# ecmwf/anemoi-models

Hardware: AMD Instinct MI355X
Metric: mesh-node updates/sec (fwd step) (higher is better)
Workload: dtype bf16; 1 GPU; N320->ico-6, 16 GT blocks, 1024 ch, batch 1, 2 x 90 input vars -> 80 output vars, full encoder+processor+decoder forward; mesh_nodes=40962, grid_nodes=542080, processor_blocks=16, rollout_steps=1, parallelism=single GPU, device=AMD Radeon Graphics

## Files before the change

anemoi_models_amd/_lib.py:

```python

from __future__ import annotations

import ctypes
import os
from ctypes import c_char_p
from ctypes import c_float
from ctypes import c_int
from ctypes import c_int64
from ctypes import c_uint32
from ctypes import c_void_p

import torch

_PKG_DIR = os.path.dirname(os.path.abspath(__file__))
LIB_PATH = os.path.join(_PKG_DIR, "lib", "libanemoi_amd.so")

ANEMOI_OK = 0
ANEMOI_ERR_INVALID = 1
ANEMOI_ERR_UNSUPPORTED = 2
ANEMOI_ERR_LAUNCH = 3

F32 = 0
BF16 = 1

ACT_NONE, ACT_GELU, ACT_SILU, ACT_RELU = 0, 1, 2, 3
ACT_CODES = {"Identity": ACT_NONE, "GELU": ACT_GELU, "SiLU": ACT_SILU, "ReLU": ACT_RELU}

ABI_VERSION = 43


class GtBlockArgs(ctypes.Structure):

    _fields_ = [
        ("struct_bytes", c_int64), ("n_dst", c_int64),
        ("dtype", ctypes.c_int32), ("C", ctypes.c_int32), ("H", ctypes.c_int32), ("up", ctypes.c_int32),
        ("hidden", ctypes.c_int32), ("act", ctypes.c_int32), ("k_proj", ctypes.c_int32), ("n_in", ctypes.c_int32),
        ("eps_mlp", c_float), ("eps_out", c_float),
        ("x", c_void_p), ("ldx", c_int64), ("x_stats", c_void_p),
        ("w_in", c_void_p), ("b_in", c_void_p), ("cs_in", c_void_p),
        ("sq", c_void_p), ("ld_sq", c_int64),
        ("q", c_void_p), ("k", c_void_p), ("v", c_void_p), ("x_r", c_void_p), ("u", c_void_p),
        ("ldq", c_int64), ("ldkv", c_int64), ("ldr", c_int64), ("ldu", c_int64),
        ("edge_attr", c_void_p), ("rowptr", c_void_p), ("col", c_void_p),
        ("att", c_void_p), ("ld_att", c_int64),
        ("w_proj", c_void_p), ("b_proj", c_void_p), ("res", c_void_p), ("ld_res", c_int64), ("y", c_void_p),
        ("y_stats", c_void_p),
        ("w_fc1", c_void_p), ("b_fc1", c_void_p), ("cs_fc1", c_void_p), ("h", c_void_p),
        ("w_fc2", c_void_p), ("b_fc2", c_void_p), ("out", c_void_p), ("out_stats", c_void_p),
        ("stats_ws", c_void_p), ("stats_ws_bytes", c_int64),
        ("run_ptr", c_void_p), ("run_perm", c_void_p), ("n_runs", c_int64),
        ("sched", c_void_p), ("sched_slots", ctypes.c_int32), ("sched_steps", ctypes.c_int32), ("n_src", c_int64),
        ("run_dst", c_void_p), ("n_edges", c_int64),
        ("tile_hdr", c_void_p), ("tile_dst", c_void_p), ("tile_src", c_void_p), ("tile_slot", c_void_p), ("tile_xcd", c_void_p),
        ("tile_max_per_xcd", ctypes.c_int32), ("tile_src_cap", ctypes.c_int32), ("tile_edge_cap", ctypes.c_int32),
        ("tile_pad", ctypes.c_int32),
    ]

class TfmBlockArgs(ctypes.Structure):

    _fields_ = [
        ("struct_bytes", c_int64), ("rows", c_int64),
        ("dtype", ctypes.c_int32), ("B", ctypes.c_int32), ("S", ctypes.c_int32), ("C", ctypes.c_int32), ("H", ctypes.c_int32),
        ("hidden", ctypes.c_int32), ("act", ctypes.c_int32), ("window", ctypes.c_int32),
        ("eps1", c_float), ("eps2", c_float),
        ("dropout_p", c_float), ("dropout_seed", c_uint32), ("dropout_seed_dev", c_void_p),
        ("dropout_h0", ctypes.c_int32), ("dropout_h_total", ctypes.c_int32),
        ("x", c_void_p), ("ldx", c_int64),
        ("ln1_w", c_void_p), ("ln1_b", c_void_p), ("ln2_w", c_void_p), ("ln2_b", c_void_p),
        ("w_qkv", c_void_p), ("b_qkv", c_void_p), ("w_proj", c_void_p), ("b_proj", c_void_p),
        ("w_fc1", c_void_p), ("b_fc1", c_void_p), ("w_fc2", c_void_p), ("b_fc2", c_void_p),
        ("h_ln", c_void_p), ("qkv", c_void_p), ("att", c_void_p), ("y", c_void_p), ("h", c_void_p),
        ("mhsa_ws", c_void_p), ("out", c_void_p),
    ]


SIGNATURES = {
    "anemoi_abi_version": (c_int, []),
    "anemoi_build_info": (ctypes.c_char_p, []),
    "anemoi_last_error": (c_char_p, []),
    "anemoi_layer_norm": (c_int, [c_int, c_void_p, c_int64, c_void_p, c_void_p, c_void_p, c_int64, c_int64, c_int,
                                  c_float, c_void_p]),
    "anemoi_layer_norm_residual": (c_int, [c_int, c_void_p, c_int64, c_void_p, c_void_p, c_void_p, c_int64, c_void_p, c_int64,
                                           c_int64, c_int, c_float, c_void_p]),
    "anemoi_layer_norm_stats": (c_int, [c_int, c_void_p, c_int64, c_void_p, c_void_p, c_void_p, c_int64, c_void_p, c_int64,
                                        c_int, c_float, c_void_p]),
    "anemoi_linear": (c_int, [c_int, c_int, c_void_p, c_int64, c_void_p, c_void_p, c_void_p, c_int64, c_void_p,
                              c_int64, c_int64, c_int, c_int, c_int, c_void_p]),
    "anemoi_linear_stats": (c_int, [c_int, c_void_p, c_int64, c_void_p, c_void_p, c_void_p, c_void_p, c_void_p, c_int64,
                                    c_void_p, c_int64, c_int64, c_int, c_int, c_void_p, c_int64, c_float, c_void_p,
                                    c_void_p]),
    "anemoi_row_stats": (c_int, [c_int, c_void_p, c_int64, c_void_p, c_int64, c_int, c_float, c_void_p]),
    "anemoi_linear_ln": (c_int, [c_int, c_int, c_void_p, c_int64, c_void_p, c_void_p, c_void_p, c_void_p, c_void_p,
                                 c_int64, c_void_p, c_int64, c_int64, c_int, c_int, c_int, c_void_p]),
    "anemoi_edge_attr_csr": (c_int, [c_void_p, c_int, c_void_p, c_int, c_int64, c_void_p, c_void_p, c_int, c_int,
                                     c_int64, c_void_p]),
    "anemoi_gt_edge_attention_folded": (c_int, [c_int, c_void_p, c_int64, c_void_p, c_void_p, c_int64, c_void_p,
                                                c_int64, c_void_p, c_int64, c_void_p, c_int, c_void_p, c_void_p,
                                                c_void_p, c_int64, c_void_p, c_int64, c_int, c_int, c_void_p]),
    "anemoi_gt_edge_attention_folded_runs": (c_int, [c_int, c_void_p, c_int64, c_void_p, c_void_p, c_int64, c_void_p,
                                                     c_int64, c_void_p, c_int64, c_void_p, c_int, c_void_p, c_void_p,
                                                     c_void_p, c_void_p, c_int64, c_void_p, c_int64, c_void_p, c_int64, c_int,
                                                     c_int, c_void_p]),
    "anemoi_gt_edge_attention_folded_groups": (c_int, [c_int, c_void_p, c_int64, c_void_p, c_void_p, c_int64, c_void_p,
                                                       c_int64, c_void_p, c_int64, c_void_p, c_int, c_void_p, c_void_p,
                                                       c_void_p, c_void_p, c_void_p, c_int64, c_int64, c_void_p, c_int64,
                                                       c_void_p, c_int64, c_int, c_int, c_void_p]),
    "anemoi_edge_schedule_shape": (c_int, [c_int, c_int64, c_int, c_void_p, c_void_p]),
    "anemoi_gt_edge_attention_folded_sched": (c_int, [c_int, c_void_p, c_int64, c_void_p, c_void_p, c_int64, c_void_p,
                                                      c_int64, c_void_p, c_int64, c_void_p, c_int, c_void_p, c_void_p,
                                                      c_void_p, c_int, c_int, c_int64, c_int64, c_void_p, c_int64, c_void_p,
                                                      c_int64, c_int, c_int, c_void_p]),
    "anemoi_gt_edge_attention_folded_tiles": (c_int, [c_int, c_void_p, c_int64, c_void_p, c_void_p, c_int64, c_void_p,
                                                      c_int64, c_void_p, c_int64, c_void_p, c_int, c_void_p, c_void_p,
                                                      c_void_p, c_void_p, c_void_p, c_void_p, c_void_p, c_int, c_int, c_int,
                                                      c_int64, c_int64, c_void_p, c_int64, c_void_p, c_int64, c_int, c_int,
                                                      c_void_p]),
    "anemoi_linear_dual": (c_int, [c_int, c_void_p, c_int64, c_void_p, c_void_p, c_void_p, c_int64, c_void_p, c_int64,
                                   c_int64, c_int, c_int, c_int, c_void_p]),
    "anemoi_linear_actgrad": (c_int, [c_int, c_void_p, c_int64, c_void_p, c_void_p, c_int64, c_void_p, c_int64, c_int64,
                                      c_int, c_int, c_int, c_void_p]),
    "anemoi_gt_conv": (c_int, [c_int, c_void_p, c_int64, c_void_p, c_void_p, c_int64, c_void_p, c_int64, c_void_p, c_int64,
                               c_void_p, c_void_p, c_void_p, c_int64, c_void_p, c_int64, c_int, c_int, c_float, c_uint32,
                               c_void_p, c_void_p]),
    "anemoi_gt_conv_backward_dst": (c_int, [c_int, c_void_p, c_int64, c_void_p, c_void_p, c_int64, c_void_p, c_int64,
                                            c_void_p, c_int64, c_void_p, c_void_p, c_void_p, c_void_p, c_void_p, c_void_p,
                                            c_void_p, c_int64, c_int64, c_int, c_int, c_float, c_uint32, c_void_p,
                                            c_void_p]),
    "anemoi_gt_conv_backward_src": (c_int, [c_int, c_void_p, c_int64, c_void_p, c_int64, c_void_p, c_void_p, c_void_p,
                                            c_void_p, c_void_p, c_void_p, c_void_p, c_void_p, c_int64, c_void_p, c_int64,
                                            c_int64, c_int, c_int, c_float, c_uint32, c_void_p, c_void_p]),
    "anemoi_gt_edge_attention": (c_int, [c_int, c_void_p, c_int64, c_void_p, c_void_p, c_int64, c_void_p, c_int64,
                                         c_void_p, c_int, c_int, c_void_p, c_void_p, c_void_p, c_void_p, c_void_p,
                                         c_int64, c_int64, c_int, c_int, c_void_p]),
    "anemoi_gather_add_act": (c_int, [c_int, c_void_p, c_int64, c_void_p, c_int64, c_void_p, c_int64, c_void_p, c_void_p,
                                      c_void_p, c_int64, c_int64, c_int, c_int, c_void_p]),
    "anemoi_segment_sum": (c_int, [c_int, c_void_p, c_int64, c_void_p, c_void_p, c_int64, c_int64, c_int, c_void_p]),
    "anemoi_segment_sum_cat": (c_int, [c_int, c_void_p, c_int64, c_void_p, c_void_p, c_int64, c_void_p, c_int64, c_int64,
                                       c_int, c_void_p]),
    "anemoi_mhsa_workspace_bytes": (c_int64, [c_int, c_int, c_int, c_int, c_int]),
    "anemoi_mhsa": (c_int, [c_int, c_void_p, c_int64, c_void_p, c_int64, c_void_p, c_void_p, c_int, c_int, c_int, c_int,
                            c_int, c_float, c_uint32, c_void_p, c_int, c_int, c_void_p]),
    "anemoi_mhsa_backward_workspace_bytes": (c_int64, [c_int, c_int, c_int, c_int, c_int]),
    "anemoi_mhsa_backward": (c_int, [c_int, c_void_p, c_int64, c_void_p, c_int64, c_void_p, c_int64, c_void_p, c_void_p,
                                     c_void_p, c_int64, c_void_p, c_int, c_int, c_int, c_int, c_int, c_float, c_uint32,
                                     c_void_p, c_int, c_int, c_void_p]),
    "anemoi_assemble_nodes": (c_int, [c_int, c_void_p, c_int, c_int, c_int, c_int64, c_int, c_void_p, c_int,
                                      c_void_p, c_int, c_void_p, c_int64, c_void_p, c_void_p, c_void_p]),
    "anemoi_finalize_output": (c_int, [c_void_p, c_int, c_void_p, c_int, c_int, c_int, c_int64, c_int, c_void_p,
                                       c_void_p, c_void_p, c_void_p, c_void_p, c_void_p]),
    "anemoi_assemble_node_rows": (c_int, [c_int, c_void_p, c_int, c_int64, c_int, c_void_p, c_int, c_void_p, c_int,
                                          c_void_p, c_int64, c_void_p, c_int64, c_void_p, c_void_p, c_void_p]),
# ... 96 lines not shown
```

anemoi_models_amd/csrc/elementwise.hip:

```cpp
#include <cstdlib>

#include "common.hpp"

namespace anemoi {

template <typename T>
__device__ __forceinline__ float round_to(float v);
template <>
__device__ __forceinline__ float round_to<float>(float v) { return v; }
template <>
__device__ __forceinline__ float round_to<bf16_t>(float v) { return bf16_to_f32(f32_to_bf16(v)); }

template <typename T, int VEC, int ITEMS>
__global__ __launch_bounds__(256) void layer_norm_kernel(const T* __restrict__ x, int64_t ldx,
                                                         const float* __restrict__ gamma,
                                                         const float* __restrict__ beta, T* __restrict__ y,
                                                         int64_t ldy, int64_t rows, int C, float eps,
                                                         float2* __restrict__ stats, const T* __restrict__ res = nullptr,
                                                         int64_t ldr = 0) {
  const int lane = threadIdx.x & 63;
  const int64_t row = (int64_t)blockIdx.x * 4 + (threadIdx.x >> 6);
  if (row >= rows) return;
  const T* xr = x + row * ldx;
  float v[ITEMS][VEC];
// ... 747 lines not shown
  hipLaunchKernelGGL(advance_input_kernel, dim3(flat_grid(total)), dim3(256), 0, as_stream(stream), x, B, T, Ens, G,
                     V_in, y, V_out, forcing, F, colmap);
  return check_launch("anemoi_advance_input");
}

static int finalize_output_impl(float* y, int V_out, const float* x, int B, int T, int Ens, int64_t G, int V_in,
                                const int32_t* src, const float* in_mul, const float* in_add, const float* out_mul,
                                const float* out_add, const int64_t* rows, int64_t n_rows, anemoi_stream_t stream) {
  ANEMOI_REQUIRE(y && x && src && B > 0 && T > 0 && Ens > 0 && G >= 0 && V_in > 0 && V_out > 0, ANEMOI_ERR_INVALID,
                 "anemoi_finalize_output: bad argument");
  ANEMOI_REQUIRE((in_mul == nullptr) == (in_add == nullptr) && (out_mul == nullptr) == (out_add == nullptr),
                 ANEMOI_ERR_INVALID, "anemoi_finalize_output: mul and add come together");
  const int64_t total = (rows != nullptr ? n_rows : (int64_t)B * Ens * G) * V_out;
  if (total == 0) return ANEMOI_OK;
  if (!force_idx64() && total < ((int64_t)1 << 31) - ((int64_t)1 << 24))
    hipLaunchKernelGGL(finalize_output_kernel<true>, dim3(flat_grid(total)), dim3(256), 0, as_stream(stream), y, V_out, x, B,
                       T, Ens, G, V_in, src, in_mul, in_add, out_mul, out_add, rows, n_rows);
  else
    hipLaunchKernelGGL(finalize_output_kernel<false>, dim3(flat_grid(total)), dim3(256), 0, as_stream(stream), y, V_out, x, B,
                       T, Ens, G, V_in, src, in_mul, in_add, out_mul, out_add, rows, n_rows);
  return check_launch("anemoi_finalize_output");
}

int anemoi_finalize_output(float* y, int V_out, const float* x, int B, int T, int Ens, int64_t G, int V_in,
                           const int32_t* src, const float* in_mul, const float* in_add, const float* out_mul,
                           const float* out_add, anemoi_stream_t stream) {
  return finalize_output_impl(y, V_out, x, B, T, Ens, G, V_in, src, in_mul, in_add, out_mul, out_add, nullptr, 0, stream);
}

int anemoi_finalize_output_rows(float* y, int V_out, const float* x, int T, int64_t G, int V_in, const int32_t* src,
                                const int64_t* rows, int64_t n_rows, const float* in_mul, const float* in_add,
                                const float* out_mul, const float* out_add, anemoi_stream_t stream) {
  ANEMOI_REQUIRE(n_rows >= 0 && (rows != nullptr || n_rows == 0), ANEMOI_ERR_INVALID,
                 "anemoi_finalize_output_rows: null row list");
  if (n_rows == 0) return ANEMOI_OK;
  return finalize_output_impl(y, V_out, x, 1, T, 1, G, V_in, src, in_mul, in_add, out_mul, out_add, rows, n_rows, stream);
}

int anemoi_bound_output(float* y, int V_out, int64_t rows, int n_ops, const int32_t* op_col, const float* op_lo,
                        const float* op_hi, const int32_t* op_mul, int n_fin, const int32_t* fin_col,
                        const float* fin_mul, const float* fin_add, anemoi_stream_t stream) {
  ANEMOI_REQUIRE(y && V_out > 0 && rows >= 0 && n_ops >= 0 && n_fin >= 0, ANEMOI_ERR_INVALID,
                 "anemoi_bound_output: bad argument");
  ANEMOI_REQUIRE(n_ops == 0 || (op_col && op_lo && op_hi && op_mul), ANEMOI_ERR_INVALID,
                 "anemoi_bound_output: null op list");
  ANEMOI_REQUIRE(n_fin == 0 || (fin_col && fin_mul && fin_add), ANEMOI_ERR_INVALID,
                 "anemoi_bound_output: null de-normalisation list");
  if (rows == 0 || (n_ops == 0 && n_fin == 0)) return ANEMOI_OK;
  hipLaunchKernelGGL(bound_output_kernel, dim3(flat_grid(rows)), dim3(256), 0, as_stream(stream), y, V_out, rows, n_ops,
                     op_col, op_lo, op_hi, op_mul, n_fin, fin_col, fin_mul, fin_add);
  return check_launch("anemoi_bound_output");
}

int anemoi_abi_version(void) { return 43; }

#ifndef ANEMOI_HIPCC_VERSION
#define ANEMOI_HIPCC_VERSION "unknown (built without anemoi_models_amd/_build.py)"
#endif
const char* anemoi_build_info(void) { return "gfx950; " ANEMOI_HIPCC_VERSION; }

const char* anemoi_last_error(void) { return err_buf(); }

}
```

anemoi_models_amd/layers/block.py:

```python

from __future__ import annotations

import os
from abc import ABC
from abc import abstractmethod
from typing import Optional

import torch
from torch import Tensor
from torch import nn

from .. import ops
from .. import runtime
from .. import training
from ..runtime import EdgePlan
from .conv import GraphConv
from .conv import GraphTransformerConv
from .mlp import MLP
from .mlp import NativeSequential
from .mlp import activation_class
from .mlp import fused_activation_name
from .mlp import linear_native


# ... 522 lines not shown
    ):
        if _group_size(model_comm_group) > 1:
            assert batch_size == 1, "Only batch size of 1 is supported when model is sharded across GPUs"
            return self._sharded(x, edge_attr, edge_index, shapes, batch_size, model_comm_group, size), edge_attr
        if training.wants_grad(self, x, edge_attr):
            return training.gt_processor_block(self, x, edge_attr, edge_index, size)
        dtype = runtime.compute_dtype(x)
        n = x.shape[0]
        if size is not None and tuple(size) != (n, n):
            raise ValueError(f"Encountered tensor with size {n} in dimension 0, but expected size {tuple(size)}")
        plan, ea = self._edge_inputs(edge_attr, edge_index, n, n, dtype)
        return self.native(_as_compute(x, dtype), ea, plan), edge_attr


class GraphTransformerMapperBlock(GraphTransformerBaseBlock):

    def __init__(
        self,
        in_channels: int,
        hidden_dim: int,
        out_channels: int,
        edge_dim: int,
        num_heads: int = 16,
        bias: bool = True,
        activation: str = "GELU",
        num_chunks: int = 1,
        update_src_nodes: bool = False,
        **kwargs,
    ) -> None:
        super().__init__(
            in_channels=in_channels, hidden_dim=hidden_dim, out_channels=out_channels, edge_dim=edge_dim,
            num_heads=num_heads, bias=bias, activation=activation, num_chunks=num_chunks,
            update_src_nodes=update_src_nodes, **kwargs,
        )
        self.layer_norm2 = nn.LayerNorm(in_channels)

    mx_node_mlp = True

    def native(self, x_src: Tensor, x_dst: Tensor, edge_attr_csr: Tensor, plan: EdgePlan, num_chunks: int = 1,
               halo=None, out_stats_eps: Optional[float] = None):
        dtype = x_dst.dtype
        self._check_channels(dtype)
        mx = runtime.mxfp8_enabled(dtype) and self.mx_node_mlp
        if mx:
            self._mx_check(self.node_dst_mlp[1].in_features if isinstance(self.node_dst_mlp[1], nn.Linear) else 0, halo)
        c = self.num_heads * self.out_channels_conv
        h_dst = x_dst.h if isinstance(x_dst, EmbeddedRows) else x_dst
        if isinstance(x_src, EmbeddedRows) and x_src.h is None and self.update_src_nodes:
            raise ValueError("update_src_nodes needs the embedded source rows")
        kv_layers, sq_layers = [self.lin_key, self.lin_value], [self.lin_self, self.lin_query]
        kv_args = ("kv", lambda: self._cat_linear("kv", kv_layers, dtype), lambda: self._cat_rows(kv_layers),
                   [l.weight for l in kv_layers] + [l.bias for l in kv_layers])
        xs = self._ln_begin(self.layer_norm1, x_src)
        if halo is None:
            kv = self._ln_linear(xs, *kv_args)
        else:
            n_own = x_src.shape[0]
            kv = torch.empty((n_own + halo.n_recv, 2 * c), dtype=dtype, device=x_src.device)
            self._ln_linear(xs, *kv_args, out=kv[:n_own])
            pending = halo.start(kv, n_own)
        del xs
        xd = self._ln_begin(self.layer_norm2, x_dst)
        up = self.fold_width(dtype)
        if up is not None:
            wp, bp = self._folded_out(dtype, up)
            sq = self._ln_linear(xd, "squ", lambda: self._folded_in("squ", sq_layers, dtype, up),
                                 lambda: self._folded_rows(sq_layers, up),
                                 self._fold_params(sq_layers))
            del xd
            if halo is not None:
                halo.finish(pending)
            if num_chunks <= 1 and not self.update_src_nodes and not mx:
                done = self._block_tail(sq[:, c:2 * c], kv[:, :c], kv[:, c:], sq[:, :c], sq[:, 2 * c:], edge_attr_csr, plan,
                                        h_dst, up, out_stats_eps)
                if done is not None:
                    return (x_src.h if isinstance(x_src, EmbeddedRows) else x_src), done
            att = folded_edge_phase(sq[:, c:2 * c], kv[:, :c], kv[:, c:], sq[:, :c], sq[:, 2 * c:], edge_attr_csr, plan,
                                    self.num_heads, up, ld_out=wp.shape[1])
        else:
            if halo is not None:
                raise NotImplementedError("node-partitioned blocks need the folded edge kernel")
            wp, bp = self._cat_linear("proj", [self.projection], dtype)
            we, be = self._edge_params()
            sq = self._ln_linear(xd, "sq", lambda: self._cat_linear("sq", sq_layers, dtype),
                                 lambda: self._cat_rows(sq_layers),
                                 [l.weight for l in sq_layers] + [l.bias for l in sq_layers])
            del xd
            att = self.conv.fused(sq[:, c:], kv[:, :c], kv[:, c:], sq[:, :c], edge_attr_csr, self.edge_dim, we, be,
                                  plan, self.num_heads)
        del sq, kv
        y = runtime.linear(att, wp, bp, residual=h_dst,
                       stats_eps=self._mlp_ln_eps("dst", dtype) if num_chunks <= 1 else None)
        del att
        if mx:
            new_dst = self._mx_node_mlp(y, "dst", num_chunks)
        else:
            new_dst = self._node_mlp(y, "dst", num_chunks, out_stats_eps=out_stats_eps)
        if isinstance(x_src, EmbeddedRows):
            x_src = x_src.h
        new_src = self._node_mlp(x_src, "src", num_chunks) if self.update_src_nodes else x_src
        return new_src, new_dst

    def _sharded(self, x, edge_attr: Tensor, edge_index: Tensor, shapes: tuple, batch_size: int, model_comm_group, size=None):
        from .. import autograd

        x_src, x_dst = x
        dtype = runtime.compute_dtype(x_dst)
        x_src, x_dst = _as_compute(x_src, dtype), _as_compute(x_dst, dtype)
        ln1, ln2 = self.layer_norm1, self.layer_norm2
        hs = autograd.layer_norm(x_src, ln1.weight, ln1.bias, ln1.eps)
        hd = autograd.layer_norm(x_dst, ln2.weight, ln2.bias, ln2.eps)
        x_r = autograd.linear(hd, self.lin_self.weight, self.lin_self.bias)
        q = autograd.linear(hd, self.lin_query.weight, self.lin_query.bias)
        k = autograd.linear(hs, self.lin_key.weight, self.lin_key.bias)
        v = autograd.linear(hs, self.lin_value.weight, self.lin_value.bias)
        e = autograd.linear(_as_compute(edge_attr, dtype), self.lin_edge.weight, self.lin_edge.bias)
        q, k, v, e = self.shard_qkve_heads(q, k, v, e, shapes, batch_size, model_comm_group)
        out = self.conv(q, k, v, e, edge_index, size=size)
        out = self.shard_output_seq(out, shapes, batch_size, model_comm_group)
        out = autograd.linear(out + x_r, self.projection.weight, self.projection.bias, "Identity", x_dst)
        new_src = training.sequential(self.node_src_mlp, x_src, residual=x_src) if self.update_src_nodes else x_src
        return new_src, training.sequential(self.node_dst_mlp, out, residual=out)

    def forward(
        self,
        x,
        edge_attr: Tensor,
        edge_index: Tensor,
        shapes: tuple,
        batch_size: int,
        model_comm_group=None,
        size=None,
    ):
        if _group_size(model_comm_group) > 1:
            assert batch_size == 1, "Only batch size of 1 is supported when model is sharded across GPUs"
            return self._sharded(x, edge_attr, edge_index, shapes, batch_size, model_comm_group, size), edge_attr
        if training.wants_grad(self, x[0], x[1], edge_attr):
            return training.gt_mapper_block(self, x, edge_attr, edge_index, size)
        x_src, x_dst = x
        dtype = runtime.compute_dtype(x_dst)
        n_src, n_dst = x_src.shape[0], x_dst.shape[0]
        if size is not None and tuple(size) != (n_src, n_dst):
            raise ValueError(f"Encountered tensors with sizes {(n_src, n_dst)}, but expected size {tuple(size)}")
        plan, ea = self._edge_inputs(edge_attr, edge_index, n_src, n_dst, dtype)
        num_chunks = self.num_chunks if self.training else inference_num_chunks()
        new_src, new_dst = self.native(_as_compute(x_src, dtype), _as_compute(x_dst, dtype), ea, plan, num_chunks)
        return (new_src if self.update_src_nodes else x[0], new_dst), edge_attr


class GraphConvBaseBlock(BaseBlock, ABC):
    def __init__(
        self,
        in_channels: int,
        out_channels: int,
        mlp_extra_layers: int = 0,
# ... 304 lines not shown
```

anemoi_models_amd/ops.py:

```python

from __future__ import annotations

from typing import NamedTuple
from typing import Optional

import torch
from torch import Tensor

from . import _lib

_DT = {torch.float32: _lib.F32, torch.bfloat16: _lib.BF16}

PROFILE: Optional[list] = None


class _Timed:
    __slots__ = ("name", "work", "start")

    def __init__(self, name: str, **work) -> None:
        self.name, self.work, self.start = name, work, None

    def __enter__(self):
        if PROFILE is not None:
            self.start = torch.cuda.Event(enable_timing=True)
# ... 387 lines not shown
        edge_attr = torch.zeros((1, up), dtype=torch.float32, device=q.device)
    alg_bytes = (2 * n_dst + 2 * k.shape[0]) * c * q.element_size() + col.shape[0] * 52 + (n_dst + 1) * 4
    fused_bytes = alg_bytes + n_dst * ((0 if x_r is None else c) + 2 * num_heads * up) * q.element_size()
    with _Timed("gt_edge_attention", bytes=alg_bytes, fused_bytes=fused_bytes, n_dst=n_dst, n_src=k.shape[0], edges=col.shape[0]):
        if runs is not None and len(runs) == 3:
            grp_ptr, grp_perm, grp_dst = runs
            _dev(grp_ptr, grp_perm, grp_dst)
            if (grp_ptr.dtype != torch.int32 or grp_perm.dtype != torch.int32 or grp_dst.dtype != torch.int32
                    or grp_perm.shape[0] != n_dst or grp_dst.shape[0] != n_dst):
                raise ValueError("gt_edge_attention_folded: runs = (int32 grp_ptr [n_groups + 1], int32 grp_perm [n_dst], "
                                 "int32 grp_dst [n_dst])")
            st = _lib.load().anemoi_gt_edge_attention_folded_groups(
                dtype_code(q.dtype), q.data_ptr(), _ld(q), k.data_ptr(), v.data_ptr(), _ld(_rows(k)), _ptr(x_r),
                0 if x_r is None else _ld(_rows(x_r)), u.data_ptr(), _ld(_rows(u)), edge_attr.data_ptr(), up,
                rowptr.data_ptr(), col.data_ptr(), grp_ptr.data_ptr(), grp_dst.data_ptr(), grp_perm.data_ptr(),
                grp_ptr.shape[0] - 1, _rows(k).shape[0], out.data_ptr(), _ld(_rows(out)), _ptr(lse), n_dst, c, num_heads,
                _stream())
        elif runs is not None:
            run_ptr, perm = runs
            _dev(run_ptr, perm)
            if run_ptr.dtype != torch.int32 or perm.dtype != torch.int32 or perm.shape[0] != run_ptr.shape[0] - 1:
                raise ValueError("gt_edge_attention_folded: runs = (int32 run_ptr [n_runs + 1], int32 perm [n_runs])")
            st = _lib.load().anemoi_gt_edge_attention_folded_runs(
                dtype_code(q.dtype), q.data_ptr(), _ld(q), k.data_ptr(), v.data_ptr(), _ld(_rows(k)), _ptr(x_r),
                0 if x_r is None else _ld(_rows(x_r)), u.data_ptr(), _ld(_rows(u)), edge_attr.data_ptr(), up,
                rowptr.data_ptr(), col.data_ptr(), run_ptr.data_ptr(), perm.data_ptr(), run_ptr.shape[0] - 1,
                out.data_ptr(), _ld(_rows(out)), _ptr(lse), n_dst, c, num_heads, _stream())
        elif tiles is not None:
            _dev(tiles.hdr, tiles.dst, tiles.src, tiles.slot, tiles.xcd)
            st = _lib.load().anemoi_gt_edge_attention_folded_tiles(
                dtype_code(q.dtype), q.data_ptr(), _ld(q), k.data_ptr(), v.data_ptr(), _ld(_rows(k)), _ptr(x_r),
                0 if x_r is None else _ld(_rows(x_r)), u.data_ptr(), _ld(_rows(u)), edge_attr.data_ptr(), up,
                rowptr.data_ptr(), col.data_ptr(), tiles.hdr.data_ptr(), tiles.dst.data_ptr(), tiles.src.data_ptr(),
                tiles.slot.data_ptr(), tiles.xcd.data_ptr(), tiles.max_tiles_per_xcd, tiles.src_cap, tiles.edge_cap,
                _rows(k).shape[0], col.shape[0], out.data_ptr(), _ld(_rows(out)), _ptr(lse), n_dst, c, num_heads, _stream())
        elif sched is not None:
            _dev(sched)
            if sched.dtype != torch.int32 or sched.dim() != 3 or sched.shape[0] != 8 or not sched.is_contiguous():
                raise ValueError("gt_edge_attention_folded: sched = contiguous int32 [8, slots, steps]")
            st = _lib.load().anemoi_gt_edge_attention_folded_sched(
                dtype_code(q.dtype), q.data_ptr(), _ld(q), k.data_ptr(), v.data_ptr(), _ld(_rows(k)), _ptr(x_r),
                0 if x_r is None else _ld(_rows(x_r)), u.data_ptr(), _ld(_rows(u)), edge_attr.data_ptr(), up,
                rowptr.data_ptr(), col.data_ptr(), sched.data_ptr(), sched.shape[1], sched.shape[2], _rows(k).shape[0],
                col.shape[0], out.data_ptr(), _ld(_rows(out)), _ptr(lse), n_dst, c, num_heads, _stream())
        else:
            st = _lib.load().anemoi_gt_edge_attention_folded(
                dtype_code(q.dtype), q.data_ptr(), _ld(q), k.data_ptr(), v.data_ptr(), _ld(_rows(k)), _ptr(x_r),
                0 if x_r is None else _ld(_rows(x_r)), u.data_ptr(), _ld(_rows(u)), edge_attr.data_ptr(), up,
                rowptr.data_ptr(), col.data_ptr(), out.data_ptr(), _ld(_rows(out)), _ptr(lse), n_dst, c, num_heads, _stream())
    _lib.check(st, "anemoi_gt_edge_attention_folded")
    return out


def gt_conv(q: Tensor, k: Tensor, v: Tensor, edges_csr: Tensor, rowptr: Tensor, col: Tensor, num_heads: int,
            x_r: Optional[Tensor] = None, lse: Optional[Tensor] = None, dropout_p: float = 0.0, dropout_seed: int = 0,
            seed_dev: Optional[Tensor] = None) -> Tensor:
    if not 0.0 <= dropout_p <= 1.0:
        raise ValueError(f"dropout probability has to be between 0 and 1, but got {dropout_p}")
    _dev(q, k, v, edges_csr, rowptr, col, x_r, lse)
    n_dst, c = _rows(q).shape
    if _ld(_rows(k)) != _ld(_rows(v)):
        raise ValueError("gt_conv: k and v must share their leading dimension")
    if rowptr.dtype != torch.int32 or col.dtype != torch.int32 or rowptr.shape[0] != n_dst + 1:
        raise ValueError("gt_conv: rowptr/col must be int32 with rowptr of length n_dst + 1")
    if edges_csr.shape[0] != col.shape[0] or edges_csr.dtype != q.dtype:
        raise ValueError("gt_conv: edges must be [E, C] in the activation dtype")
    out = torch.empty((n_dst, c), dtype=q.dtype, device=q.device)
    if col.shape[0] == 0:
        if lse is not None:
            lse.fill_(float("-inf"))
        return out.zero_() if x_r is None else out.copy_(x_r)
    alg_bytes = (2 * n_dst + 2 * k.shape[0] + col.shape[0]) * c * q.element_size() + col.shape[0] * 4 + (n_dst + 1) * 4
    with _Timed("gt_conv", bytes=alg_bytes, n_dst=n_dst, n_src=k.shape[0], edges=col.shape[0]):
        st = _lib.load().anemoi_gt_conv(dtype_code(q.dtype), q.data_ptr(), _ld(q), k.data_ptr(), v.data_ptr(), _ld(_rows(k)),
                                        edges_csr.data_ptr(), _ld(_rows(edges_csr)), _ptr(x_r),
                                        0 if x_r is None else _ld(_rows(x_r)), rowptr.data_ptr(), col.data_ptr(),
                                        out.data_ptr(), _ld(out), _ptr(lse), n_dst, c, num_heads, float(dropout_p),
                                        int(dropout_seed) & 0xFFFFFFFF, _seed_dev_ptr(seed_dev, q), _stream())
    _lib.check(st, "anemoi_gt_conv")
    return out


def gather_add_act(t: Tensor, p_dst: Tensor, p_src: Tensor, dst: Tensor, src: Tensor, act: str = "Identity",
                   out: Optional[Tensor] = None) -> Tensor:
    _dev(t, p_dst, p_src, dst, src, out)
    e, c = _rows(t).shape
    if out is None:
        out = torch.empty((e, c), dtype=t.dtype, device=t.device)
    if e == 0:
        return out
    if dst.dtype != torch.int32 or src.dtype != torch.int32 or dst.shape[0] != e or src.shape[0] != e:
        raise ValueError("gather_add_act: dst / src must be int32 [E]")
    with _Timed("gather_add_act", bytes=(2 * e + p_dst.shape[0] + p_src.shape[0]) * c * t.element_size() + 8 * e):
        st = _lib.load().anemoi_gather_add_act(dtype_code(t.dtype), t.data_ptr(), _ld(t), p_dst.data_ptr(),
                                               _ld(_rows(p_dst)), p_src.data_ptr(), _ld(_rows(p_src)), dst.data_ptr(),
                                               src.data_ptr(), out.data_ptr(), _ld(_rows(out)), e, c,
                                               _lib.ACT_CODES[act], _stream())
    _lib.check(st, "anemoi_gather_add_act")
    return out


def segment_sum(v: Tensor, rowptr: Tensor, out: Optional[Tensor] = None, cat_with: Optional[Tensor] = None) -> Tensor:
    _dev(v, rowptr, out, cat_with)
    n_dst = rowptr.shape[0] - 1
    c = _rows(v).shape[1]
    if cat_with is not None:
# ... 438 lines not shown
```

include/anemoi_amd.h:

```cpp
#ifndef ANEMOI_AMD_H
#define ANEMOI_AMD_H

#include <stdint.h>

#ifdef __cplusplus
extern "C" {
#endif

#define ANEMOI_OK 0
#define ANEMOI_ERR_INVALID 1
#define ANEMOI_ERR_UNSUPPORTED 2
#define ANEMOI_ERR_LAUNCH 3

#define ANEMOI_F32 0
#define ANEMOI_BF16 1

#define ANEMOI_ACT_NONE 0
#define ANEMOI_ACT_GELU 1
#define ANEMOI_ACT_SILU 2
#define ANEMOI_ACT_RELU 3

typedef void* anemoi_stream_t;

int anemoi_abi_version(void);
const char* anemoi_build_info(void);
const char* anemoi_last_error(void);

int anemoi_layer_norm(int dtype, const void* x, int64_t ldx, const float* gamma, const float* beta, void* y,
                      int64_t ldy, int64_t rows, int C, float eps, anemoi_stream_t stream);

int anemoi_layer_norm_residual(int dtype, const void* x, int64_t ldx, const float* gamma, const float* beta,
                               const void* residual, int64_t ldr, void* y, int64_t ldy, int64_t rows, int C, float eps,
                               anemoi_stream_t stream);

int anemoi_layer_norm_stats(int dtype, const void* x, int64_t ldx, const float* gamma, const float* beta, void* y,
                            int64_t ldy, float* stats, int64_t rows, int C, float eps, anemoi_stream_t stream);

int anemoi_linear(int dtype, int out_dtype, const void* x, int64_t ldx, const void* w, const float* bias,
                  const void* residual, int64_t ldr, void* y, int64_t ldy, int64_t M, int N, int K, int act,
                  anemoi_stream_t stream);

int anemoi_row_stats(int dtype, const void* x, int64_t ldx, float* stats, int64_t rows, int C, float eps,
                     anemoi_stream_t stream);

int anemoi_linear_ln(int dtype, int out_dtype, const void* x, int64_t ldx, const void* w, const float* bias,
                     const float* colsum, const float* stats, const void* residual, int64_t ldr, void* y, int64_t ldy,
                     int64_t M, int N, int K, int act, anemoi_stream_t stream);

int anemoi_linear_stats(int dtype, const void* x, int64_t ldx, const void* w, const float* bias, const float* colsum,
                        const float* stats_in, const void* residual, int64_t ldr, void* y, int64_t ldy, int64_t M, int N,
                        int K, void* workspace, int64_t workspace_bytes, float eps, float* stats_out,
                        anemoi_stream_t stream);

int anemoi_edge_attr_csr(const float* a0, int d0, const float* a1, int d1, int64_t rows0, const int32_t* perm,
                         float* out, int ld_out, int one_col, int64_t n_edges, anemoi_stream_t stream);

int anemoi_gt_edge_attention(int dtype, const void* q, int64_t ldq, const void* k, const void* v, int64_t ldkv,
                             const void* x_r, int64_t ldr, const float* edge_attr, int ea_ld, int edge_dim,
                             const float* w_edge, const float* b_edge, const int32_t* rowptr, const int32_t* col,
                             void* out, int64_t ldo, int64_t n_dst, int C, int H, anemoi_stream_t stream);

int anemoi_gt_edge_attention_folded(int dtype, const void* q, int64_t ldq, const void* k, const void* v, int64_t ldkv,
                                    const void* x_r, int64_t ldr, const void* u, int64_t ldu, const float* edge_attr,
                                    int up, const int32_t* rowptr, const int32_t* col, void* out, int64_t ldo, float* lse,
                                    int64_t n_dst, int C, int H, anemoi_stream_t stream);

int anemoi_gt_edge_attention_folded_runs(int dtype, const void* q, int64_t ldq, const void* k, const void* v, int64_t ldkv,
                                         const void* x_r, int64_t ldr, const void* u, int64_t ldu, const float* edge_attr,
                                         int up, const int32_t* rowptr, const int32_t* col, const int32_t* run_ptr,
                                         const int32_t* run_perm, int64_t n_runs, void* out, int64_t ldo, float* lse,
                                         int64_t n_dst, int C, int H, anemoi_stream_t stream);

int anemoi_gt_edge_attention_folded_groups(int dtype, const void* q, int64_t ldq, const void* k, const void* v, int64_t ldkv,
                                           const void* x_r, int64_t ldr, const void* u, int64_t ldu, const float* edge_attr,
                                           int up, const int32_t* rowptr, const int32_t* col, const int32_t* grp_ptr,
                                           const int32_t* grp_dst, const int32_t* grp_perm, int64_t n_groups, int64_t n_src,
                                           void* out, int64_t ldo, float* lse, int64_t n_dst, int C, int H,
                                           anemoi_stream_t stream);

int anemoi_edge_schedule_shape(int dtype, int64_t n_dst, int C, int* slots, int* steps);
int anemoi_gt_edge_attention_folded_sched(int dtype, const void* q, int64_t ldq, const void* k, const void* v, int64_t ldkv,
                                          const void* x_r, int64_t ldr, const void* u, int64_t ldu, const float* edge_attr,
                                          int up, const int32_t* rowptr, const int32_t* col, const int32_t* sched, int slots,
                                          int steps, int64_t n_src, int64_t n_edges, void* out, int64_t ldo, float* lse,
                                          int64_t n_dst, int C, int H, anemoi_stream_t stream);

int anemoi_gt_edge_attention_folded_tiles(int dtype, const void* q, int64_t ldq, const void* k, const void* v, int64_t ldkv,
                                          const void* x_r, int64_t ldr, const void* u, int64_t ldu, const float* edge_attr,
                                          int up, const int32_t* rowptr, const int32_t* col, const int32_t* tile_hdr,
                                          const int32_t* tile_dst, const int32_t* tile_src, const uint8_t* tile_slot,
                                          const int32_t* tile_xcd, int max_tiles_per_xcd, int src_cap, int edge_cap,
                                          int64_t n_src, int64_t n_edges, void* out, int64_t ldo, float* lse, int64_t n_dst,
                                          int C, int H, anemoi_stream_t stream);

int anemoi_gt_conv(int dtype, const void* q, int64_t ldq, const void* k, const void* v, int64_t ldkv, const void* edges,
                   int64_t lde, const void* x_r, int64_t ldr, const int32_t* rowptr, const int32_t* col, void* out,
                   int64_t ldo, float* lse, int64_t n_dst, int C, int H, float dropout_p, uint32_t dropout_seed,
                   const void* dropout_seed_dev, anemoi_stream_t stream);
int anemoi_gt_conv_backward_dst(int dtype, const void* q, int64_t ldq, const void* k, const void* v, int64_t ldkv,
                                const void* edges, int64_t lde, const void* dout, int64_t ldd, const float* lse,
                                const int32_t* rowptr, const int32_t* col, float* alpha, float* w, float* dsum, void* dq,
                                int64_t lddq, int64_t n_dst, int C, int H, float dropout_p, uint32_t dropout_seed,
                                const void* dropout_seed_dev, anemoi_stream_t stream);
int anemoi_gt_conv_backward_src(int dtype, const void* q, int64_t ldq, const void* dout, int64_t ldd, const float* alpha,
                                const float* w, const float* dsum, const int32_t* rowptr_t, const int32_t* eid_t,
                                const int32_t* dst_t, void* dk, void* dv, int64_t ldg, void* dedges, int64_t ldde,
                                int64_t n_src, int C, int H, float dropout_p, uint32_t dropout_seed,
                                const void* dropout_seed_dev, anemoi_stream_t stream);

int anemoi_assemble_nodes(int dtype, const float* x, int B, int T, int Ens, int64_t G, int V, const float* latlons,
                          int n_ll, const float* trainable, int n_tr, void* out, int64_t ldo, const float* in_mul,
                          const float* in_add, anemoi_stream_t stream);

int anemoi_assemble_node_rows(int dtype, const float* x, int T, int64_t G, int V, const float* latlons, int n_ll,
                              const float* trainable, int n_tr, const int64_t* rows, int64_t n_rows, void* out,
                              int64_t ldo, const float* in_mul, const float* in_add, anemoi_stream_t stream);

int anemoi_finalize_output(float* y, int V_out, const float* x, int B, int T, int Ens, int64_t G, int V_in,
// ... 179 lines not shown
```

Before: 19.19 million mesh-node updates/s.

## Attend over raw source rows instead of materializing projected keys and values

```diff
diff --git a/anemoi_models_amd/_lib.py b/anemoi_models_amd/_lib.py
--- a/anemoi_models_amd/_lib.py
+++ b/anemoi_models_amd/_lib.py
@@ -26,7 +26,7 @@
 ACT_NONE, ACT_GELU, ACT_SILU, ACT_RELU = 0, 1, 2, 3
 ACT_CODES = {"Identity": ACT_NONE, "GELU": ACT_GELU, "SiLU": ACT_SILU, "ReLU": ACT_RELU}
 
-ABI_VERSION = 43
+ABI_VERSION = 44
 
 
 class GtBlockArgs(ctypes.Structure):
@@ -97,6 +97,9 @@
     "anemoi_gt_edge_attention_folded": (c_int, [c_int, c_void_p, c_int64, c_void_p, c_void_p, c_int64, c_void_p,
                                                 c_int64, c_void_p, c_int64, c_void_p, c_int, c_void_p, c_void_p,
                                                 c_void_p, c_int64, c_void_p, c_int64, c_int, c_int, c_void_p]),
+    "anemoi_gt_edge_attention_raw": (c_int, [c_void_p, c_int64, c_void_p, c_int64, c_void_p, c_void_p, c_int64, c_void_p,
+                                             c_int, c_void_p, c_void_p, c_void_p, c_int64, c_void_p, c_int64, c_int64,
+                                             c_int, c_int, c_int, c_int, c_void_p]),
     "anemoi_gt_edge_attention_folded_runs": (c_int, [c_int, c_void_p, c_int64, c_void_p, c_void_p, c_int64, c_void_p,
                                                      c_int64, c_void_p, c_int64, c_void_p, c_int, c_void_p, c_void_p,
                                                      c_void_p, c_void_p, c_int64, c_void_p, c_int64, c_void_p, c_int64, c_int,
diff --git a/anemoi_models_amd/csrc/edge_attention_raw.hip b/anemoi_models_amd/csrc/edge_attention_raw.hip
--- /dev/null
+++ b/anemoi_models_amd/csrc/edge_attention_raw.hip
@@ -0,0 +1,234 @@
+#include <cmath>
+
+#include "common.hpp"
+
+namespace anemoi {
+
+typedef __attribute__((ext_vector_type(8))) __bf16 rbf16x8_t;
+typedef __attribute__((ext_vector_type(4))) short rs16x4_t;
+typedef __attribute__((ext_vector_type(4))) float rf32x4_t;
+typedef uint32_t ru32x4_t __attribute__((ext_vector_type(4)));
+typedef uint32_t ru32x2_t __attribute__((ext_vector_type(2)));
+
+struct EdgeRawParams {
+  const bf16_t* qt;
+  const bf16_t* x;
+  const float* stats;
+  const bf16_t* u;
+  bf16_t* g;
+  bf16_t* t;
+  int64_t ldqt, ldx, ldu, ldg, ldt;
+  int64_t n_dst;
+  int sum_col;
+  float scale;
+};
+
+template <int KS, int UP>
+__global__ __launch_bounds__(256, (KS == 256 || UP > 8) ? 2 : 3) void gt_edge_attention_raw_kernel(const EdgeRawParams p,
+                                                                    const float* __restrict__ attr_,
+                                                                    const int32_t* __restrict__ rowptr_,
+                                                                    const int32_t* __restrict__ col_) {
+  constexpr int T = KS / 32;
+  constexpr int NT = KS / 16;
+  constexpr int PITCH = KS * 2 + 16;
+  __shared__ __attribute__((aligned(16))) unsigned char image[4][16 * PITCH];
+
+  const int lane = threadIdx.x & 63;
+  const int wib = __builtin_amdgcn_readfirstlane((int)(threadIdx.x >> 6));
+  const int r16 = lane & 15, g4 = lane >> 4;
+  const int xcd = blockIdx.x & 7;
+  const int64_t n0 = p.n_dst * xcd / 8, n1 = p.n_dst * (xcd + 1) / 8;
+  const int64_t node = n0 + (int64_t)(blockIdx.x >> 3) * 4 + wib;
+  if (node >= n1) return;
+  unsigned char* tile = image[wib];
+
+  const int e_begin = __builtin_amdgcn_readfirstlane(rowptr_[node]);
+  const int e_end = __builtin_amdgcn_readfirstlane(rowptr_[node + 1]);
+
+  rbf16x8_t qb[T];
+  {
+    const bf16_t* qrow = p.qt + node * p.ldqt + r16 * KS + g4 * 8;
+#pragma unroll
+    for (int t = 0; t < T; ++t) qb[t] = __builtin_bit_cast(rbf16x8_t, *reinterpret_cast<const ru32x4_t*>(qrow + t * 32));
+  }
+  float u[UP];
+  {
+    const uint32_t* uw = reinterpret_cast<const uint32_t*>(p.u + node * p.ldu + r16 * UP);
+#pragma unroll
+    for (int a = 0; a < UP / 2; ++a) {
+      const uint32_t w = uw[a];
+      u[2 * a] = __uint_as_float(w << 16);
+      u[2 * a + 1] = __uint_as_float(w & 0xffff0000u);
+    }
+  }
+
+  float m = -INFINITY, lsum = 0.f;
+  float tacc[UP];
+  rf32x4_t acc[NT];
+#pragma unroll
+  for (int a = 0; a < UP; ++a) tacc[a] = 0.f;
+#pragma unroll
+  for (int n = 0; n < NT; ++n) acc[n] = rf32x4_t{0.f, 0.f, 0.f, 0.f};
+
+  for (int e0 = e_begin; e0 < e_end; e0 += 16) {
+    ru32x4_t xa[T];
+    {
+      const int ea = min(e0 + r16, e_end - 1);
+      const bf16_t* xrow = p.x + (int64_t)col_[ea] * p.ldx + g4 * 8;
+#pragma unroll
+      for (int t = 0; t < T; ++t) xa[t] = *reinterpret_cast<const ru32x4_t*>(xrow + t * 32);
+    }
+    float rs[4], at[4][UP];
+    bool valid[4];
+#pragma unroll
+    for (int q = 0; q < 4; ++q) {
+      const int eq = e0 + g4 * 4 + q;
+      valid[q] = eq < e_end;
+      const int ec = valid[q] ? eq : e_end - 1;
+      rs[q] = p.stats[2 * (int64_t)col_[ec]];
+      const float4* ap = reinterpret_cast<const float4*>(attr_ + (int64_t)ec * UP);
+#pragma unroll
+      for (int a = 0; a < UP / 4; ++a) {
+        const float4 v = ap[a];
+        at[q][4 * a] = v.x; at[q][4 * a + 1] = v.y; at[q][4 * a + 2] = v.z; at[q][4 * a + 3] = v.w;
+      }
+    }
+
+    rf32x4_t s4 = {0.f, 0.f, 0.f, 0.f};
+#pragma unroll
+    for (int t = 0; t < T; ++t)
+      s4 = __builtin_amdgcn_mfma_f32_16x16x32_bf16(__builtin_bit_cast(rbf16x8_t, xa[t]), qb[t], s4, 0, 0, 0);
+#pragma unroll
+    for (int t = 0; t < T; ++t) *reinterpret_cast<ru32x4_t*>(tile + r16 * PITCH + t * 64 + g4 * 16) = xa[t];
+
+    float s[4], cmax = -INFINITY;
+#pragma unroll
+    for (int q = 0; q < 4; ++q) {
+      float ua = 0.f;
+#pragma unroll
+      for (int a = 0; a < UP; ++a) ua = fmaf(u[a], at[q][a], ua);
+      s[q] = valid[q] ? fmaf(rs[q], s4[q], ua) * p.scale : -INFINITY;
+      cmax = fmaxf(cmax, s[q]);
+    }
+    cmax = fmaxf(cmax, __shfl_xor(cmax, 16, 64));
+    cmax = fmaxf(cmax, __shfl_xor(cmax, 32, 64));
+    const float mb = fmaxf(m, cmax);
+    const float corr = __expf(m - mb);
+    float pe[4], psum = 0.f;
+#pragma unroll
+    for (int q = 0; q < 4; ++q) {
+      pe[q] = valid[q] ? __expf(s[q] - mb) : 0.f;
+      psum += pe[q];
+    }
+    lsum = fmaf(lsum, corr, psum);
+#pragma unroll
+    for (int a = 0; a < UP; ++a) {
+      float ta = tacc[a] * corr;
+#pragma unroll
+      for (int q = 0; q < 4; ++q) ta = fmaf(pe[q], at[q][a], ta);
+      tacc[a] = ta;
+    }
+#pragma unroll
+    for (int n = 0; n < NT; ++n) acc[n] *= corr;
+    m = mb;
+    const rs16x4_t pb = __builtin_bit_cast(
+        rs16x4_t, ru32x2_t{pack_bf16x2(pe[0] * rs[0], pe[1] * rs[1]), pack_bf16x2(pe[2] * rs[2], pe[3] * rs[3])});
+
+    __builtin_amdgcn_fence(__ATOMIC_RELEASE, "wavefront");
+    __builtin_amdgcn_wave_barrier();
+    __builtin_amdgcn_fence(__ATOMIC_ACQUIRE, "wavefront");
+    const int tr_off = (g4 * 4 + (r16 >> 2)) * PITCH + (r16 & 3) * 8;
+#pragma unroll
+    for (int n = 0; n < NT; ++n) {
+      const rs16x4_t xt = __builtin_amdgcn_ds_read_tr16_b64_v4i16(
+          (__attribute__((address_space(3))) rs16x4_t*)(tile + tr_off + n * 32));
+      acc[n] = __builtin_amdgcn_mfma_f32_16x16x16bf16_1k(xt, pb, acc[n], 0, 0, 0);
+    }
+    __builtin_amdgcn_fence(__ATOMIC_RELEASE, "wavefront");
+    __builtin_amdgcn_wave_barrier();
+  }
+
+  lsum += __shfl_xor(lsum, 16, 64);
+  lsum += __shfl_xor(lsum, 32, 64);
+  const float inv = 1.0f / (lsum + 1e-16f);
+  const float asum = lsum * inv;
+#pragma unroll
+  for (int a = 0; a < UP; ++a) {
+    float ta = tacc[a];
+    ta += __shfl_xor(ta, 16, 64);
+    ta += __shfl_xor(ta, 32, 64);
+    tacc[a] = ta * inv;
+  }
+  if (g4 == 0) {
+    uint32_t* tw = reinterpret_cast<uint32_t*>(p.t + node * p.ldt + r16 * UP);
+#pragma unroll
+    for (int a = 0; a < UP / 2; ++a) tw[a] = pack_bf16x2(tacc[2 * a], tacc[2 * a + 1]);
+  }
+  bf16_t* grow = p.g + node * p.ldg + r16 * KS + g4 * 4;
+#pragma unroll
+  for (int n = 0; n < NT; ++n) {
+    float o[4];
+#pragma unroll
+    for (int j = 0; j < 4; ++j) o[j] = (n * 16 + g4 * 4 + j == p.sum_col) ? asum : acc[n][j] * inv;
+    *reinterpret_cast<ru32x2_t*>(grow + n * 16) = ru32x2_t{pack_bf16x2(o[0], o[1]), pack_bf16x2(o[2], o[3])};
+  }
+}
+
+template <int KS, int UP>
+static void launch_raw(const EdgeRawParams& p, const float* attr, const int32_t* rowptr, const int32_t* col,
+                       hipStream_t st) {
+  const int64_t per_xcd = (p.n_dst + 7) / 8;
+  const int64_t bpx = (per_xcd + 3) / 4;
+  hipLaunchKernelGGL((gt_edge_attention_raw_kernel<KS, UP>), dim3((unsigned)(8 * bpx)), dim3(256), 0, st, p, attr, rowptr,
+                     col);
+}
+
+template <int KS>
+static bool dispatch_raw(const EdgeRawParams& p, int up, const float* attr, const int32_t* rowptr, const int32_t* col,
+                         hipStream_t st) {
+  switch (up) {
+    case 4: launch_raw<KS, 4>(p, attr, rowptr, col, st); return true;
+    case 8: launch_raw<KS, 8>(p, attr, rowptr, col, st); return true;
+    case 12: launch_raw<KS, 12>(p, attr, rowptr, col, st); return true;
+    case 16: launch_raw<KS, 16>(p, attr, rowptr, col, st); return true;
+    default: return false;
+  }
+}
+
+}
+
+extern "C" int anemoi_gt_edge_attention_raw(const void* qt, int64_t ldqt, const void* x, int64_t ldx,
+                                            const float* src_stats, const void* u, int64_t ldu,
+                                            const float* edge_attr, int up, const int32_t* rowptr, const int32_t* col,
+                                            void* g, int64_t ldg, void* t, int64_t ldt, int64_t n_dst, int H, int Ks,
+                                            int D, int sum_col, anemoi_stream_t stream) {
+  using namespace anemoi;
+  ANEMOI_REQUIRE(qt && x && src_stats && u && g && t && rowptr, ANEMOI_ERR_INVALID,
+                 "anemoi_gt_edge_attention_raw: null pointer");
+  ANEMOI_REQUIRE(n_dst >= 0 && D > 0 && sum_col >= -1 && sum_col < Ks, ANEMOI_ERR_INVALID,
+                 "anemoi_gt_edge_attention_raw: bad argument");
+  ANEMOI_REQUIRE(H == 16 && (Ks == 64 || Ks == 128 || Ks == 256) && up >= 4 && up <= 16 && up % 4 == 0, ANEMOI_ERR_UNSUPPORTED,
+                 "anemoi_gt_edge_attention_raw: needs 16 heads, 64, 128 or 256 raw columns, up in {4, 8, 12, 16} (H=%d, Ks=%d, up=%d)",
+                 H, Ks, up);
+  ANEMOI_REQUIRE(ldqt >= (int64_t)H * Ks && ldg >= (int64_t)H * Ks && ldx >= Ks && ldu >= (int64_t)H * up &&
+                     ldt >= (int64_t)H * up,
+                 ANEMOI_ERR_INVALID, "anemoi_gt_edge_attention_raw: leading dimension too small");
+  if (n_dst == 0) return ANEMOI_OK;
+  ANEMOI_REQUIRE(col != nullptr && edge_attr != nullptr, ANEMOI_ERR_INVALID,
+                 "anemoi_gt_edge_attention_raw: null edge arrays");
+  const bool aligned = (uintptr_t)qt % 16 == 0 && (uintptr_t)x % 16 == 0 && (uintptr_t)g % 16 == 0 &&
+                       (uintptr_t)u % 8 == 0 && (uintptr_t)t % 8 == 0 && (uintptr_t)edge_attr % 16 == 0 &&
+                       ldqt % 8 == 0 && ldx % 8 == 0 && ldg % 8 == 0 && ldu % 4 == 0 && ldt % 4 == 0;
+  ANEMOI_REQUIRE(aligned, ANEMOI_ERR_UNSUPPORTED, "anemoi_gt_edge_attention_raw: operands must be 16-byte aligned");
+  EdgeRawParams p;
+  p.qt = static_cast<const bf16_t*>(qt); p.x = static_cast<const bf16_t*>(x); p.stats = src_stats;
+  p.u = static_cast<const bf16_t*>(u); p.g = static_cast<bf16_t*>(g); p.t = static_cast<bf16_t*>(t);
+  p.ldqt = ldqt; p.ldx = ldx; p.ldu = ldu; p.ldg = ldg; p.ldt = ldt;
+  p.n_dst = n_dst; p.sum_col = sum_col;
+  p.scale = 1.0f / sqrtf((float)D);
+  const bool ok = Ks == 256   ? dispatch_raw<256>(p, up, edge_attr, rowptr, col, as_stream(stream))
+                  : Ks == 128 ? dispatch_raw<128>(p, up, edge_attr, rowptr, col, as_stream(stream))
+                              : dispatch_raw<64>(p, up, edge_attr, rowptr, col, as_stream(stream));
+  ANEMOI_REQUIRE(ok, ANEMOI_ERR_UNSUPPORTED, "anemoi_gt_edge_attention_raw: up=%d", up);
+  return check_launch("anemoi_gt_edge_attention_raw");
+}
diff --git a/anemoi_models_amd/csrc/elementwise.hip b/anemoi_models_amd/csrc/elementwise.hip
--- a/anemoi_models_amd/csrc/elementwise.hip
+++ b/anemoi_models_amd/csrc/elementwise.hip
@@ -823,7 +823,7 @@
   return check_launch("anemoi_bound_output");
 }
 
-int anemoi_abi_version(void) { return 43; }
+int anemoi_abi_version(void) { return 44; }
 
 #ifndef ANEMOI_HIPCC_VERSION
 #define ANEMOI_HIPCC_VERSION "unknown (built without anemoi_models_amd/_build.py)"
diff --git a/anemoi_models_amd/layers/block.py b/anemoi_models_amd/layers/block.py
--- a/anemoi_models_amd/layers/block.py
+++ b/anemoi_models_amd/layers/block.py
@@ -598,6 +598,9 @@
         kv_args = ("kv", lambda: self._cat_linear("kv", kv_layers, dtype), lambda: self._cat_rows(kv_layers),
                    [l.weight for l in kv_layers] + [l.bias for l in kv_layers])
         xs = self._ln_begin(self.layer_norm1, x_src)
+        raw = None if (halo is not None or num_chunks > 1 or mx) else self._raw_source_weights(x_src, dtype)
+        if raw is not None:
+            return x_src.h, self._native_raw_sources(x_src, xs[1], x_dst, h_dst, edge_attr_csr, plan, raw, out_stats_eps)
         if halo is None:
             kv = self._ln_linear(xs, *kv_args)
         else:
@@ -647,6 +650,66 @@
         new_src = self._node_mlp(x_src, "src", num_chunks) if self.update_src_nodes else x_src
         return new_src, new_dst
 
+    RAW_ROWS_DEFAULT = "1"
+
+    def _raw_source_weights(self, x_src, dtype):
+        h, d = self.num_heads, self.out_channels_conv
+        if (not isinstance(x_src, EmbeddedRows) or x_src.h is not None or self.update_src_nodes
+                or dtype != torch.bfloat16 or not x_src.x_aug.is_cuda
+                or os.environ.get("ANEMOI_AMD_EDGE_RAW", self.RAW_ROWS_DEFAULT) == "0"):
+            return None
+        ks, k_in = x_src.x_aug.shape[1], x_src.emb.in_features
+        sum_col = ks - 1 if x_src.one_col != ks - 1 else ks - 2
+        if self.fold_width(dtype) is None or h != 16 or ks not in (64, 128, 256) or sum_col < k_in:
+            return None
+        kv_layers = [self.lin_key, self.lin_value]
+        ln, emb = self.layer_norm1, x_src.emb
+
+        def build():
+            f, b, _ = runtime.fold_embedded_layer_norm(*self._cat_rows(kv_layers), ln.weight, ln.bias, emb.weight,
+                                                       emb.bias, ks, x_src.one_col, torch.float32)
+            c = h * d
+            w_qt = f[:c].view(h, d, ks).transpose(1, 2)
+            w_g = f[c:].view(h, d, ks).clone()
+            w_g[:, :, sum_col] = b[c:].view(h, d)
+            if d % ops.k_multiple(dtype) != 0:
+                w_qt, w_g = torch.block_diag(*w_qt), torch.block_diag(*w_g)
+            return w_qt.to(dtype).contiguous(), w_g.to(dtype).contiguous(), sum_col
+
+        return self._packed.get(("kv", "rawrows", dtype, ks, x_src.one_col, x_src._tag),
+                                [l.weight for l in kv_layers] + [l.bias for l in kv_layers]
+                                + [ln.weight, ln.bias, emb.weight, emb.bias], build)
+
+    def _native_raw_sources(self, x_src, src_stats: Tensor, x_dst, h_dst: Tensor, edge_attr_csr: Tensor, plan, raw,
+                            out_stats_eps: Optional[float]) -> Tensor:
+        dtype = x_dst.dtype
+        c, h = self.num_heads * self.out_channels_conv, self.num_heads
+        w_qt, w_g, sum_col = raw
+        up = self.fold_width(dtype)
+        sq_layers = [self.lin_self, self.lin_query]
+        wp, bp = self._folded_out(dtype, up)
+        sq = self._ln_linear(self._ln_begin(self.layer_norm2, x_dst), "squ",
+                             lambda: self._folded_in("squ", sq_layers, dtype, up),
+                             lambda: self._folded_rows(sq_layers, up), self._fold_params(sq_layers))
+        per_head = w_qt.dim() == 3
+        qt = ops.linear_heads(sq[:, c:2 * c], w_qt) if per_head else runtime.linear(sq[:, c:2 * c], w_qt)
+        att = torch.empty((sq.shape[0], wp.shape[1]), dtype=dtype, device=sq.device)
+        if wp.shape[1] > c + h * up:
+            att[:, c + h * up:].zero_()
+        g = ops.gt_edge_attention_raw(qt, x_src.x_aug, src_stats, sq[:, 2 * c:2 * c + h * up], edge_attr_csr, plan.rowptr,
+                                      plan.col, h, self.out_channels_conv, up, sum_col, att[:, c:c + h * up])
+        del qt
+        if per_head:
+            ops.linear_heads(g, w_g, out=att[:, :c])
+            ops.add(att[:, :c], sq[:, :c], out=att[:, :c])
+        else:
+            runtime.linear(g, w_g, residual=sq[:, :c], out=att[:, :c])
+        del g
+        del sq
+        y = runtime.linear(att, wp, bp, residual=h_dst, stats_eps=self._mlp_ln_eps("dst", dtype))
+        del att
+        return self._node_mlp(y, "dst", 1, out_stats_eps=out_stats_eps)
+
     def _sharded(self, x, edge_attr: Tensor, edge_index: Tensor, shapes: tuple, batch_size: int, model_comm_group, size=None):
         from .. import autograd
 
diff --git a/anemoi_models_amd/ops.py b/anemoi_models_amd/ops.py
--- a/anemoi_models_amd/ops.py
+++ b/anemoi_models_amd/ops.py
@@ -463,6 +463,65 @@
     return out
 
 
+def linear_heads(x: Tensor, w: Tensor, out: Optional[Tensor] = None) -> Tensor:
+    _dev(x, w, out)
+    _rows(x)
+    if w.dim() != 3 or w.dtype != x.dtype or not w.is_contiguous():
+        raise ValueError("linear_heads: weight must be contiguous [H, N, K] in the activation dtype")
+    h, n, k = w.shape
+    if x.shape[1] < h * k:
+        raise ValueError(f"linear_heads: x has {x.shape[1]} columns, {h} heads of {k} expected")
+    if out is None:
+        out = torch.empty((x.shape[0], h * n), dtype=x.dtype, device=x.device)
+    if _rows(out).shape[1] < h * n or out.dtype != x.dtype or out.shape[0] != x.shape[0]:
+        raise ValueError("linear_heads: out must be [M, >= H*N] in the activation dtype")
+    m = x.shape[0]
+    if m == 0:
+        return out
+    code = dtype_code(x.dtype)
+    with _Timed("linear", flops=2 * m * h * n * k, bytes=(m * h * (k + n) + h * n * k) * x.element_size(), m=m, n=h * n,
+                k=k, heads=h):
+        st = _lib.load().anemoi_linear_batched(code, code, x.data_ptr(), _ld(x), k, w.data_ptr(), n * k, out.data_ptr(),
+                                               _ld(out), n, h, m, n, k, _stream())
+    _lib.check(st, "anemoi_linear_batched")
+    return out
+
+
+def gt_edge_attention_raw(qt: Tensor, x_raw: Tensor, src_stats: Tensor, u: Tensor, edge_attr: Tensor, rowptr: Tensor,
+                          col: Tensor, num_heads: int, head_dim: int, up: int, sum_col: int, t_out: Tensor,
+                          g: Optional[Tensor] = None) -> Tensor:
+    _dev(qt, x_raw, src_stats, u, edge_attr, rowptr, col, t_out, g)
+    n_dst, ks = _rows(qt).shape[0], _rows(x_raw).shape[1]
+    if qt.dtype != torch.bfloat16 or x_raw.dtype != torch.bfloat16 or u.dtype != torch.bfloat16 or t_out.dtype != torch.bfloat16:
+        raise NotImplementedError("gt_edge_attention_raw: bf16 only")
+    if qt.shape[1] != num_heads * ks:
+        raise ValueError(f"gt_edge_attention_raw: qt has {qt.shape[1]} columns, {num_heads} heads of {ks} expected")
+    if (src_stats.shape != (x_raw.shape[0], 2) or src_stats.dtype != torch.float32 or not src_stats.is_contiguous()):
+        raise ValueError("gt_edge_attention_raw: src_stats must be the contiguous [n_src, 2] f32 result of row_stats")
+    if rowptr.dtype != torch.int32 or col.dtype != torch.int32 or rowptr.shape[0] != n_dst + 1:
+        raise ValueError("gt_edge_attention_raw: rowptr/col must be int32 with rowptr of length n_dst + 1")
+    if edge_attr.shape[0] != col.shape[0] or (col.shape[0] > 0 and (edge_attr.shape[1] != up or
+                                                                      not edge_attr.is_contiguous())):
+        raise ValueError("gt_edge_attention_raw: edge_attr must be contiguous [E, up]")
+    if _rows(u).shape != (n_dst, num_heads * up) or _rows(t_out).shape[0] != n_dst or t_out.shape[1] < num_heads * up:
+        raise ValueError("gt_edge_attention_raw: u / t_out must be [n_dst, H*up]")
+    if g is None:
+        g = torch.empty((n_dst, num_heads * ks), dtype=qt.dtype, device=qt.device)
+    if col.shape[0] == 0:
+        col = torch.zeros(1, dtype=torch.int32, device=qt.device)
+        edge_attr = torch.zeros((1, up), dtype=torch.float32, device=qt.device)
+    alg_bytes = (col.shape[0] * (ks * 2 + 4 + up * 4 + 4) + 2 * n_dst * num_heads * ks * 2 + (n_dst + 1) * 4)
+    fused_bytes = alg_bytes + n_dst * 2 * num_heads * up * 2
+    with _Timed("gt_edge_attention", bytes=alg_bytes, fused_bytes=fused_bytes, n_dst=n_dst, n_src=x_raw.shape[0],
+                edges=col.shape[0], raw_rows=ks):
+        st = _lib.load().anemoi_gt_edge_attention_raw(
+            qt.data_ptr(), _ld(qt), x_raw.data_ptr(), _ld(x_raw), src_stats.data_ptr(), u.data_ptr(), _ld(u),
+            edge_attr.data_ptr(), up, rowptr.data_ptr(), col.data_ptr(), g.data_ptr(), _ld(_rows(g)), t_out.data_ptr(),
+            _ld(t_out), n_dst, num_heads, ks, head_dim, sum_col, _stream())
+    _lib.check(st, "anemoi_gt_edge_attention_raw")
+    return g
+
+
 def gt_conv(q: Tensor, k: Tensor, v: Tensor, edges_csr: Tensor, rowptr: Tensor, col: Tensor, num_heads: int,
             x_r: Optional[Tensor] = None, lse: Optional[Tensor] = None, dropout_p: float = 0.0, dropout_seed: int = 0,
             seed_dev: Optional[Tensor] = None) -> Tensor:
diff --git a/include/anemoi_amd.h b/include/anemoi_amd.h
--- a/include/anemoi_amd.h
+++ b/include/anemoi_amd.h
@@ -64,6 +64,11 @@
                                     const void* x_r, int64_t ldr, const void* u, int64_t ldu, const float* edge_attr,
                                     int up, const int32_t* rowptr, const int32_t* col, void* out, int64_t ldo, float* lse,
                                     int64_t n_dst, int C, int H, anemoi_stream_t stream);
+
+int anemoi_gt_edge_attention_raw(const void* qt, int64_t ldqt, const void* x, int64_t ldx, const float* src_stats,
+                                 const void* u, int64_t ldu, const float* edge_attr, int up, const int32_t* rowptr,
+                                 const int32_t* col, void* g, int64_t ldg, void* t, int64_t ldt, int64_t n_dst, int H,
+                                 int Ks, int D, int sum_col, anemoi_stream_t stream);
 
 int anemoi_gt_edge_attention_folded_runs(int dtype, const void* q, int64_t ldq, const void* k, const void* v, int64_t ldkv,
                                          const void* x_r, int64_t ldr, const void* u, int64_t ldu, const float* edge_attr,
```

Measured after the change: 19.57 million mesh-node updates/s (median of 6 runs). +2.0%, better.
